# chu-tianxiang/QuIP-for-all

Hardware: AMD Instinct MI355X
Metric: decode tokens/sec bs=1 Llama-7B E8P12 2-bit, 1xMI355X; % HBM roofline (higher is better)
Workload: dtype i8xi8->i32 (fp16 I/O); 1 GPU; Llama-2-7B E8P12 random-init, bs=1 greedy decode, 1 hipGraph replay per token, positions [5, 833) of a 2048-slot static KV cache; layers=32, hidden=4096, ffn=11008, vocab=32000, parallelism=replicas x1 (no collective on the data path)

## Files before the change

quip_for_all_amd/csrc/decode_block.hip:

```cpp
#if defined(QUIP_POLL2) || defined(QUIP_POLL2_STAGGER) || defined(QUIP_ROWS_DIRECT) || defined(QUIP_MLP_PREFETCH) || defined(QUIP_INO_EXACT) || \
    defined(QUIP_QKV_ISSUE_EARLY) || defined(QUIP_OWNER_PREDECODE) || defined(QUIP_ATT_THREADS) || defined(QUIP_OHEAD)
#error "retired A/B switch (QUIP_POLL2, _POLL2_STAGGER, _ROWS_DIRECT, _MLP_PREFETCH, _INO_EXACT, _QKV_ISSUE_EARLY, _OWNER_PREDECODE, _ATT_THREADS, _OHEAD): the alternative was measured and its code removed; DESIGN.md 4.11 (QUIP_OHEAD: 4.13) has the result and the commit that still contains it"
#endif
#include "e8p_gemv_core.hip.h"
#include "attn_query.hip.h"
#include "engine_sync.hip.h"
#include "fht_wg512x.hip.h"
#include "token_tail.hip.h"
#include "block_engine_host.hip.h"

#ifndef QUIP_PREDECODE_DOWN
#define QUIP_PREDECODE_DOWN 2
#endif
#ifndef QUIP_PREDECODE_QKV
#define QUIP_PREDECODE_QKV 2
#endif
#ifndef QUIP_ATT_STAMPS
#define QUIP_ATT_STAMPS 0
#endif
#ifndef QUIP_MLP_STAMPS
#define QUIP_MLP_STAMPS 0
#endif
#if QUIP_MLP_STAMPS
#define MSTAMP(i) BSTAMP((i) < 7 ? 18 + (i) : 21 + (i))
#else
#define MSTAMP(i) do { } while (0)
#endif
#if QUIP_ATT_STAMPS
#define ASTAMP(i) BSTAMP(18 + (i))
#else
#define ASTAMP(i) do { } while (0)
#endif
#ifndef QUIP_WAIT_STAMPS
#define QUIP_WAIT_STAMPS 0
#endif
#if (QUIP_ATT_STAMPS != 0) + (QUIP_MLP_STAMPS != 0) + (QUIP_WAIT_STAMPS != 0) > 1
#error "QUIP_ATT_STAMPS, QUIP_MLP_STAMPS and QUIP_WAIT_STAMPS share the stamp slots 18..31: one at a time"
#endif
#if QUIP_WAIT_STAMPS == 1
#define WSTAMP(i) BSTAMP((i) < 7 ? 18 + (i) : 21 + (i))
#else
#define WSTAMP(i) do { } while (0)
#endif
#ifndef QUIP_NIB_PREDECODE_QKV
#define QUIP_NIB_PREDECODE_QKV 3
#endif
#ifndef QUIP_NIB_PREDECODE_GATE
#define QUIP_NIB_PREDECODE_GATE 3
#endif
#ifndef QUIP_NIB_PREDECODE_DOWN
#define QUIP_NIB_PREDECODE_DOWN 3
#endif
#ifndef QUIP_PREDECODE_GATE
#define QUIP_PREDECODE_GATE 2
#endif

namespace quip {

namespace {

using esync::u32x2_t;
using esync::u32x4_t;

struct BlockLayer {
  const uint4* W[7];
// ... 99 lines not shown
#if QUIP_BLOCK_G8
static_assert(BLds<24>::kBytes <= 160 * 1024 && BLds<4>::kBytes <= 160 * 1024, "LDS budget");
#else
static_assert(BLds<4>::kBytes <= 160 * 1024 && BLds<24>::kBytes <= 160 * 1024 && BLds<16>::kBytes <= 160 * 1024 && BLds<64>::kBytes <= 160 * 1024 &&
              BLds<16, true>::kBytes <= 160 * 1024 && BLds<64, true>::kBytes <= 160 * 1024 && BLds<12, true>::kBytes <= 160 * 1024,
              "LDS budget");
#endif

template <int REP, bool RVQ = false, bool HI = false>
__global__ __launch_bounds__(kThreads) void decode_block_kernel(BlockArgs a) {
  static_assert(!HI || (RVQ && Lds<REP>::kD4), "HI = virtual rows of twice the width on the D4 table mode");
  constexpr bool R3 = Lds<REP>::kRvq3;
  static_assert(!R3 || (RVQ && !HI), "RVQ3B: the virtual rows of RVQ");
  using slot_t = std::conditional_t<R3, u32x3, u32x4>;
  constexpr uint32_t PB = R3 ? 12u : 16u;
  extern __shared__ __attribute__((aligned(16))) char smem[];
  using B = BLds<REP, RVQ>;
  constexpr int VM = B::VM, KV = B::KV;
  constexpr int kRowU4V = VM * kRowU4, kRowU4DV = VM * kRowU4D;
  constexpr int kRowB = kRowU4V * 16;
  using T = Lds<REP>;
  int tid = threadIdx.x, lane = tid & 63;
  const int wave = __builtin_amdgcn_readfirstlane(tid >> 6);
  const int w = blockIdx.x;
  const int mgu = w >> 7;
  int n = lane & 15, q = lane >> 4;
  uint32_t* ctl = reinterpret_cast<uint32_t*>(a.ws + kWsCtl);
  uint64_t* zbufs = reinterpret_cast<uint64_t*>(a.ws + kWsZ);
  uint64_t* inbox = reinterpret_cast<uint64_t*>(a.ws + kWsInbox);
  uint64_t* frow = reinterpret_cast<uint64_t*>(a.ws + kWsRows);
  uint64_t* pbuf = reinterpret_cast<uint64_t*>(a.ws + kWsPart);
  int dbg_on = 0;
  const bool dbg_rt = (a.dbg_layer & 0x10000) != 0;
#define BSTAMP(i) do { if (dbg_on && tid == 0) a.dbg[w * 32 + (i)] = dbg_rt ? __builtin_amdgcn_s_memrealtime() : __builtin_amdgcn_s_memtime(); } while (0)

  slot_t qa[NSLOT], qb[NSLOT];
  uint32_t vo_row, vo_q[3], vo_gu[G8 ? 7 : FRB], vo_d[G8 ? 4 : 3], vo_d2b, vo_dr[3];
  const int qb0 = w < 128 ? 2 * w : 128 + w, qcnt = w < 128 ? 2 : 1;
  auto qmat = [](int b) { return b < 256 ? 0 : (b < 320 ? 1 : 2); };
  auto qblk = [](int b) { return b < 256 ? b : (b < 320 ? b - 256 : b - 320); };
  uint32_t lane_c, lane_c2, lane_c3 = 0u, xlane;
  constexpr bool NIB = T::kNib;
  constexpr bool kOHead = !RVQ;
  constexpr int kPreW = NIB ? 16 : 32;
  constexpr int kUnsc = T::kD4 ? 1 : (NIB ? 5 : 2);
  NibLane nlf = {0, 0, 0u};
  auto rederive = [&]() {
    int t = threadIdx.x;
    asm volatile("" : "+v"(t));
    tid = t; lane = t & 63; n = lane & 15; q = lane >> 4;
    vo_row = (uint32_t)((w * RPW + n) * kRowU4V + wave * 8 + q) * PB;
    if constexpr (G8) {
#pragma unroll
      for (int i = 0; i < 2; ++i) {
        const int bq = qb0 + (i < qcnt ? i : 0);
        vo_q[i] = (uint32_t)((qblk(bq) * 16 + n) * kRowU4V + wave * 8 + q) * PB;
      }
      vo_q[2] = vo_q[0];
#pragma unroll
      for (int i = 0; i < 7; ++i) {
        const int r = 16 * i + n, c = r >= FK ? 1 : 0, k = r - FK * c;
        vo_gu[i] = (uint32_t)((k * FL + 2 * (w & 127) + c) * kRowU4V + wave * 8 + q) * PB;
      }
#pragma unroll
      for (int i = 0; i < 4; ++i) {
        const int sl0 = i * kWaves + wave;
        const int sl = sl0 < JD ? sl0 : 0;
        vo_d[i] = (uint32_t)(((w * RPW + n) * kRowU4D + sl * 8 + q) * 16);
      }
      vo_d2b = 0u;
    } else if constexpr (TILED) {
      static_assert(!TILED || (!RVQ && PB == 16u), "the launch-tiled layout: plain E8P12 rows");
      constexpr int C = kRowU4V / 4, CD = kRowU4D / 4;
      const uint32_t lo = (uint32_t)lane * 16u;
      vo_row = (uint32_t)((w * C + 2 * wave) * 1024) + lo;
#pragma unroll
      for (int i = 0; i < 3; ++i) vo_q[i] = (uint32_t)((((3 * w + i) & 255) * C + 2 * wave) * 1024) + lo;
// ... 162 lines not shown
    h_in = a.tail.embed + (size_t)(tk >= 0 && tk < (long long)a.tail.vocab ? tk : 0) * HID;
  }
#pragma unroll
  for (int k = 0; k < 8; ++k)
    asm volatile("global_load_ushort %0, %1, off" : "=v"(hraw[k]) : "v"(reinterpret_cast<const uint16_t*>(h_in) + tid + 512 * k) : "memory");
  {
    const BlockLayer& L0 = a.layers[0];
    if constexpr (RVQ) ISSUE_RVQ_QKV(L0); else if constexpr (G8) { ISSUE8_QKV(L0, 0); ISSUE8_QKV(L0, 1); } else { ISSUE(L0, 0); ISSUE(L0, 1); ISSUE(L0, 2); }
  }
  constexpr int NQ = RVQ ? 12 : (G8 ? 4 : 6);
  int* accs = reinterpret_cast<int*>(smem + B::kAcc);
  for (int i = tid; i < B::kAccRows * 4; i += kThreads) accs[i] = 0;
  asm volatile("s_waitcnt vmcnt(%2)" : "+v"(tsrc), "+v"(tsrc3) : "n"(9 + NQ) : "memory");
  if constexpr (NIB) fill_tables_nib(tsrc, lane, wave);
  else fill_tables_from_lane<REP>(smem, tsrc, lane, wave);
  fill_t3_from_lane<REP>(smem, tsrc3, lane, wave);
  asm volatile("s_waitcnt vmcnt(%1)" : "+v"(gen) : "n"(8 + NQ) : "memory");
  const uint32_t ebase = ((uint32_t)__builtin_amdgcn_readfirstlane((int)gen) + 1u) << 10;
  asm volatile("s_waitcnt vmcnt(%8)" : "+v"(hraw[0]), "+v"(hraw[1]), "+v"(hraw[2]), "+v"(hraw[3]), "+v"(hraw[4]), "+v"(hraw[5]),
               "+v"(hraw[6]), "+v"(hraw[7]) : "n"(NQ) : "memory");
#pragma unroll
  for (int j = 0; j < 4; ++j) hreg[j] = (hraw[2 * j] & 0xffffu) | (hraw[2 * j + 1] << 16);
  const long long pos64 = *a.pos;
  const bool pos_ok = pos64 >= 0 && pos64 < (long long)a.max_len;
  const int pos = pos_ok ? (int)pos64 : 0;
  if (tid < 2 * HD)
    reinterpret_cast<float*>(smem + B::kCs)[tid] = (tid < HD ? a.cos : a.sin - HD)[(size_t)pos * HD + tid];
  had::wg_barrier<true>();
  uint32_t hop = 0;

  float* red = reinterpret_cast<float*>(smem + B::kRed);
  int* shs = reinterpret_cast<int*>(smem + B::kRed + 256);

  auto gather = [&](auto nv_tag, auto slots, int first, uint32_t tag, uint32_t code, float (&out)[decltype(nv_tag)::value][8]) {
    constexpr int NV = decltype(nv_tag)::value;
    u32x4_t p[2 * NV];
    uint32_t spins = 0;
    const uint64_t* src = zbufs + (size_t)first * 2048 + 4 * tid;
    for (;;) {
#pragma unroll
      for (int c = 0; c < NV; ++c) {
        esync::ld16(p[2 * c], src + c * 2048);
        esync::ld16(p[2 * c + 1], src + c * 2048 + 2);
      }
      esync::drain();
      bool ok = true;
#pragma unroll
      for (int j = 0; j < 2 * NV; ++j) {
        esync::own(p[j]);
        ok = ok && p[j].y == tag && p[j].w == tag;
      }
      if (esync::spin_step(ok, spins, ctl + 1, code + (uint32_t)w)) break;
    }
#pragma unroll
    for (int c = 0; c < NV; ++c)
      had::unpack8(make_uint4(p[2 * c].x, p[2 * c].z, p[2 * c + 1].x, p[2 * c + 1].z), out[c]);
    own_slots(slots);
  };
  auto publish16 = [&](int vec, int gr0, int row0, int sh, uint32_t tag) {
    if (tid < 8) {
      const int* s3 = accs + (row0 + 2 * tid) * 4;
      const float us = unscale_of(sh, kUnsc);
      const float f0 = __builtin_fmaf((float)s3[0], 65536.f, __builtin_fmaf((float)s3[1], 256.f, (float)s3[2]));
      const float f1 = __builtin_fmaf((float)s3[4], 65536.f, __builtin_fmaf((float)s3[5], 256.f, (float)s3[6]));
      esync::st_granule(zbufs + (size_t)vec * 2048 + gr0 + tid, pack_f16(f0 * us, f1 * us), tag);
    }
  };
  auto zero_acc = [&](int row0, int rows) {
    for (int i = tid; i < rows * 4; i += kThreads) accs[row0 * 4 + i] = 0;
  };

  constexpr bool E2 = B::kTwoBuf;
  float* xbuf = reinterpret_cast<float*>(smem + B::kBuf0);
  float* xbuf1 = reinterpret_cast<float*>(smem + B::kBuf1);
  auto planes_nat = [&](const float (&v)[8], float scale, int sh, uint32_t base) {
#pragma clang fp contract(off)
    const float p2 = as_f32((uint32_t)(sh + 127) << 23);
    const float s2 = had::fmul(scale, p2);
    const float va[4] = {v[0], v[1], v[2], v[3]}, vb[4] = {v[4], v[5], v[6], v[7]};
    if constexpr (HI) {
      const float e0[4] = {v[0], v[2], 0.f, 0.f}, e1[4] = {v[4], v[6], 0.f, 0.f}, e2[4] = {v[1], v[3], 0.f, 0.f}, e3[4] = {v[5], v[7], 0.f, 0.f};
      uint32_t dg[3][4];
      hadw::digit_words_magic(e0, s2, dg[0][0], dg[1][0], dg[2][0]);
      hadw::digit_words_magic(e1, s2, dg[0][1], dg[1][1], dg[2][1]);
      hadw::digit_words_magic(e2, s2, dg[0][2], dg[1][2], dg[2][2]);
      hadw::digit_words_magic(e3, s2, dg[0][3], dg[1][3], dg[2][3]);
#pragma unroll
      for (int d = 0; d < 3; ++d)
        *reinterpret_cast<uint4*>(smem + base + d * 2 * HID + 16 * tid) = make_uint4(dg[d][0], dg[d][1], dg[d][2], dg[d][3]);
    } else if constexpr (RVQ) {
// ... 1 lines not shown
      uint32_t dg[3][4];
      hadw::digit_words_magic(va, s2r, dg[0][0], dg[1][0], dg[2][0]);
      hadw::digit_words_magic(vb, s2r, dg[0][1], dg[1][1], dg[2][1]);
      hadw::digit_words_magic(va, s2, dg[0][2], dg[1][2], dg[2][2]);
      hadw::digit_words_magic(vb, s2, dg[0][3], dg[1][3], dg[2][3]);
#pragma unroll
      for (int d = 0; d < 3; ++d)
        *reinterpret_cast<uint4*>(smem + base + d * 2 * HID + 16 * tid) = make_uint4(dg[d][0], dg[d][1], dg[d][2], dg[d][3]);
    } else {
      uint32_t dg[3][2];
      hadw::digit_words_magic(va, s2, dg[0][0], dg[1][0], dg[2][0]);
      hadw::digit_words_magic(vb, s2, dg[0][1], dg[1][1], dg[2][1]);
#pragma unroll
      for (int d = 0; d < 3; ++d) {
        if constexpr (NIB) {
          *reinterpret_cast<uint32_t*>(smem + base + d * B::PSH + 4 * tid) = dg[d][0];
          *reinterpret_cast<uint32_t*>(smem + base + d * B::PSH + B::HOH + 4 * tid) = dg[d][1];
        } else {
          *reinterpret_cast<uint2*>(smem + base + d * HID + 8 * tid) = make_uint2(dg[d][0], dg[d][1]);
        }
      }
    }
  };
  auto norm_shift = [&](float sumsq_x, float scale) -> int {
    const float bound = sqrtf(sumsq_x) * 64.f * fabsf(scale) * 1.0625f;
    return had::shift_for(bound * ((RVQ && !HI) ? fmaxf(1.f, fabsf(a.resid_scale)) : 1.f));
  };
  auto red_sum8 = [&](int at) -> float {
    float r = red[at];
#pragma unroll
    for (int i = 1; i < 8; ++i) r = had::fadd(r, red[at + i]);
    return r;
  };
  auto edge = [&](auto z_tag, auto nc_tag, auto slots, int zvec, uint32_t tag, uint32_t code, const f16* sv_prev, const f16* ln,
                  const f16* su0, const f16* su1, float sc0, float sc1, bool two, auto after_gather, auto drip1, auto drip2, int sb) {
#if QUIP_ATT_STAMPS || QUIP_MLP_STAMPS || QUIP_WAIT_STAMPS
#define ESTAMP(i) do { } while (0)
#else
#define ESTAMP(i) do { if (sb >= 0) BSTAMP(sb + (i) + ((sb == 23 && (i) >= 2) ? 3 : 0)); } while (0)
#endif
    constexpr int NC = decltype(nc_tag)::value;
    constexpr bool HAVE_Z = decltype(z_tag)::value;
    u32x4 psv, pln, psu0, psu1;
    if constexpr (HAVE_Z) psv = *reinterpret_cast<const u32x4*>(sv_prev + 8 * tid);
    if constexpr (NC > 0) {
      pln = *reinterpret_cast<const u32x4*>(ln + 8 * tid);
      psu0 = *reinterpret_cast<const u32x4*>(su0 + 8 * tid);
      psu1 = *reinterpret_cast<const u32x4*>(su1 + 8 * tid);
    }
    auto u4 = [](const u32x4& v) { return make_uint4(v.x, v.y, v.z, v.w); };
    if constexpr (HAVE_Z) {
      float v[1][8];
      gather(std::integral_constant<int, 1>{}, slots, zvec, tag, code, v);
      asm volatile("" : "+v"(psv));
      if constexpr (NC > 0) asm volatile("" : "+v"(pln), "+v"(psu0), "+v"(psu1));
      after_gather();
      ESTAMP(0);
      hadw::fwd<12, 1, true, !E2>(v, xbuf, tid);
      ESTAMP(1);
      float svf[8];
      had::unpack8(u4(psv), svf);
#pragma unroll
      for (int j = 0; j < 4; ++j) {
        const f16x2 hh = as_f16x2(hreg[j]);
        const f16 n0 = had::out_elem(v[0][2 * j], 1.f / 64.f, true, svf[2 * j], false, 0.f, true, (float)hh.x);
        const f16 n1 = had::out_elem(v[0][2 * j + 1], 1.f / 64.f, true, svf[2 * j + 1], false, 0.f, true, (float)hh.y);
        hreg[j] = (uint32_t)__builtin_bit_cast(uint16_t, n0) | ((uint32_t)__builtin_bit_cast(uint16_t, n1) << 16);
      }
      drip1();
    }
    if constexpr (NC > 0) {
      float e[8];
#pragma unroll
      for (int j = 0; j < 4; ++j) {
        const f16x2 hh = as_f16x2(hreg[j]);
        e[2 * j] = (float)hh.x;
        e[2 * j + 1] = (float)hh.y;
      }
      float ssw = 0.f;
      {
#pragma clang fp contract(off)
#pragma unroll
        for (int r = 0; r < 8; ++r) ssw = __builtin_fmaf(e[r], e[r], ssw);
      }
      had::mul8(e, u4(pln));
      const int lane_ = tid & 63;
// ... 199 lines not shown
      had::wg_barrier<true>();
      ++hop;
      const int sh_lo = shs[0], sh_hi = shs[1];
      publish16(qc_lo, qblk(qb0) * 8, 0, sh_lo, ebase | hop);
      if (qcnt == 2) publish16(qc_hi, qblk(qb0 + 1) * 8, 16, qc_hi == qc_lo ? sh_lo : sh_hi, ebase | hop);
      had::wg_barrier<true>();
      zero_acc(0, 48);
      BSTAMP(3);
      return;
    }
    {
      const uint32_t x0 = xlane + (uint32_t)((((3 * w) >> 8) == c_lo ? 0 : 1) * 3 * B::PSH);
      const uint32_t x1 = xlane + (uint32_t)((((3 * w + 1) >> 8) == c_lo ? 0 : 1) * 3 * B::PSH);
      const uint32_t x2 = xlane + (uint32_t)((((3 * w + 2) >> 8) == c_lo ? 0 : 1) * 3 * B::PSH);
      if constexpr (decltype(pre_tag)::value) run_items3_pre(std::integral_constant<int, NPQ>{}, preq, 0, x0, x1, x2, 0);
      else run_items3(0, x0, x1, x2, 0);
      if constexpr (RVQ) run_items3(3, x0 + 4096u, x1 + 4096u, x2 + 4096u, 0);
    }
    had::wg_barrier<true>();
    ++hop;
    const int sh_lo = shs[0], sh_hi = shs[1];
#pragma unroll
    for (int i = 0; i < 3; ++i) {
      const int rbq = 3 * w + i, ci = rbq >> 8;
      publish16(ci, (rbq & 255) * 8, i * 16, ci == c_lo ? sh_lo : sh_hi, ebase | hop);
    }
    had::wg_barrier<true>();
    zero_acc(0, 48);
    BSTAMP(3);
  };
  {
    rederive();
    const int c_lo = qc_lo, c_hi = qc_hi;
    edge(std::false_type{}, std::integral_constant<int, 2>{}, SLOTS(M_QKV), -1, 0u, 0u, nullptr, Ld.ln[0], Ld.su[c_lo], Ld.su[c_hi],
         Ld.sc[c_lo], Ld.sc[c_hi], c_hi != c_lo, [&]() {}, [&]() {}, [&]() {}, -1);
    uint32_t none[NPQ][kPreW];
    P1_products(std::false_type{}, none);
  }
  for (int l = 0; l < a.n_layers; ++l) {
    dbg_on = a.dbg != nullptr && l == (a.dbg_layer & 0xffff);
    rederive();
    BSTAMP(0);
    if (tid < 64)
      reinterpret_cast<uint32_t*>(smem + B::kDescN)[tid] = reinterpret_cast<const uint32_t*>(a.layers + (l + 1 < a.n_layers ? l + 1 : l))[tid];
    if constexpr (RVQ) ISSUE_RVQ_O(Ld); else ISSUE(Ld, 3);

    rederive();
    const bool split = pos >= kSplitPos;
    const int part = w & 7, nparts = split ? kParts : 1;
    const bool head_wg = part == 0;
    const int hd = w >> 3;
    if (head_wg || split) {
      float c8[8], s8[8];
      const int d0 = (tid & 15) * 8;
      constexpr int ATH = 256;
      constexpr int LPK = HD / 8, NG = ATH / LPK, U = (RVQ && !HI && !R3) ? 2 : 4;
      constexpr int NST = ATH / 64;
      const int g = (tid & (ATH - 1)) / LPK;
      const int kvh = hd / GQH;
      const f16* kc = Ld.kcache + (size_t)kvh * a.max_len * HD;
      const f16* vc = Ld.vcache + (size_t)kvh * a.max_len * HD;
      uint4 kr0[U], vr0[U], kr1[U], vr1[U];
      const attn::CachedRows<HD, U, NG> rows{kc, vc, part, nparts, pos, d0};
      if (tid < ATH) {
        rows.load_round(kr0, vr0, g);
        if (part + nparts * NG * U < pos) rows.load_round(kr1, vr1, g + NG * U);
      }
      uint32_t svp_raw = 0u;
// ... 323 lines not shown
        if constexpr (RVQ) ISSUE_RVQ_GATE_G(Ld, 2); else if constexpr (G8) ISSUE8_GU(Ld, 2); else ISSUE(Ld, 6);
        if constexpr (HI) had8::planes_scatter_hi(v[0], sco, sh, reinterpret_cast<uint8_t*>(smem + B::kArea), tid);
        else if constexpr (RVQ) had8::planes_scatter_rvq(v[0], sco, a.resid_scale, sh, reinterpret_cast<uint8_t*>(smem + B::kArea), tid);
        else if constexpr (NIB) {
#pragma clang fp contract(off)
          const float s2 = had::fmul(sco, as_f32((uint32_t)(sh + 127) << 23));
          uint8_t* pb = reinterpret_cast<uint8_t*>(smem + B::kArea) + nib_half_of(tid) * B::HOH + nib_byte_of(tid);
#pragma unroll
          for (int k = 0; k < 8; ++k) {
            const int X = (int)__builtin_rintf(v[0][k] * s2);
            const int X1 = (X + 128) >> 8;
            const int H = (X1 + 128) >> 8;
            uint8_t* p = pb + 256 * k;
            p[0] = (uint8_t)H;
            p[B::PSH] = (uint8_t)X1;
            p[2 * B::PSH] = (uint8_t)X;
          }
        }
        else had8::planes_scatter(v[0], sco, sh, reinterpret_cast<uint8_t*>(smem + B::kArea), tid);
        if (tid == 0) shs[3] = sh;
        had::wg_barrier<true>();
      }
    }
    BSTAMP(8);
    if constexpr (RVQ) {
      run_item(6, xlane, 48);
      run_item(7, xlane + 4096u, 48);
    } else {
      if constexpr (NIB) { Frag Fo; frags(xlane, Fo); add_rows(mul_pre(Bon, Fo), 48); }
      else add_rows(item_multiply(Bo, xlane), 48);
    }
    had::wg_barrier<true>();
    ++hop;
    publish16(4, w * 8, 48, shs[3], ebase | hop);
    had::wg_barrier<true>();
    zero_acc(48, 16);
    BSTAMP(9);

    rederive();
#if QUIP_PREDECODE_GATE
    uint32_t Bg[kPreG][kPreW];
    if constexpr (!RVQ) {
      esync::drain();
      own_slots(SLOTS(M_GATE));
#pragma unroll
      for (int i = 0; i < kPreG; ++i) decode_pre(i, Bg[i]);
    }
#endif
    constexpr int HPIECES = B::kHadElems / 8, NHP = (HPIECES + kThreads - 1) / kThreads, OPIECES = RPO * 3 * (FL / 8);
    static_assert(OPIECES <= kThreads, "one piece of the owner vectors per thread");
    u32x4 fim[NHP], ovec = {0u, 0u, 0u, 0u};
#pragma unroll
    for (int i = 0; i < NHP; ++i) {
      const int pi = tid + kThreads * i;
      fim[i] = reinterpret_cast<const u32x4*>(Ld.had3)[pi < HPIECES ? pi : tid];
    }
    if (w < NRO) {
      const int p = tid < OPIECES ? tid : 0;
      const int row = p / (3 * (FL / 8)), rem = p - row * (3 * (FL / 8));
      const int vsel = rem / (FL / 8), piece = rem - vsel * (FL / 8);
      const int kr = RPO * w + row < FK ? RPO * w + row : FK - 1;
      ovec = *reinterpret_cast<const u32x4*>((vsel == 0 ? Ld.sv[4] : (vsel == 1 ? Ld.sv[5] : Ld.su[6])) + (size_t)kr * FL + piece * 8);
    }
    auto land_mlp_vectors = [&]() {
#pragma unroll
      for (int i = 0; i < NHP; ++i) {
        asm volatile("" : "+v"(fim[i]));
        if (tid + kThreads * i < HPIECES) *reinterpret_cast<u32x4*>(smem + B::kHad + (tid + kThreads * i) * 16) = fim[i];
      }
      asm volatile("" : "+v"(ovec));
      if (w < NRO && tid < OPIECES) *reinterpret_cast<u32x4*>(smem + B::kStash + tid * 16) = ovec;
    };
    edge(std::true_type{}, std::integral_constant<int, 2>{}, SLOTS(M_GATE), 4, ebase | hop, 0x7000u, Ld.sv[3], Ld.ln[1], Ld.su[4 + mgu], Ld.su[4 + mgu], Ld.sc[4 + mgu], Ld.sc[4 + mgu], false,
         [&]() { land_mlp_vectors(); BSTAMP(10); if constexpr (RVQ) ISSUE_RVQ_UP_A_G(Ld, 0); else if constexpr (G8) { ISSUE8_GU(Ld, 3); ISSUE8_GU(Ld, 4); } else ISSUE(Ld, 7); },
         [&]() { if constexpr (RVQ) ISSUE_RVQ_UP_A_G(Ld, 1); else if constexpr (G8) ISSUE8_GU(Ld, 5); else ISSUE(Ld, 8); },
         [&]() { if constexpr (RVQ) ISSUE_RVQ_UP_A_G(Ld, 2); else if constexpr (G8) ISSUE8_GU(Ld, 6); else ISSUE(Ld, 9); }, 18);
    BSTAMP(11);
    MSTAMP(0);
    if constexpr (RVQ || G8) {
      esync::drain();
      own_slots(SLOTS(M_GATE | M_UP));
    }
    MSTAMP(1);
    static_assert(FRB == 3, "three row blocks per matrix");
    if constexpr (RVQ) {
      const uint32_t xu = xlane;
      run_items3(0, xlane, xlane, xlane, 64);
      ISSUE_RVQ_UP_B(Ld);
      run_items3(3, xlane + 4096u, xlane + 4096u, xlane + 4096u, 64);
      run_items3(6, xu, xu, xu, 64 + 16 * FRB);
      esync::drain();
      own_slots(SLOTS(0x007u));
      run_items3(0, xu + 4096u, xu + 4096u, xu + 4096u, 64 + 16 * FRB);
    } else {
      if constexpr (G8) {
        Frag A;
        frags(xlane, A);
#if QUIP_PREDECODE_GATE
#define PRE_G(i) ((i) < kPreG ? Bg[(i) < kPreG ? (i) : 0] : nullptr)
#else
#define PRE_G(i) nullptr
#endif
        add_rows(item_vs(std::integral_constant<int, 0>{}, PRE_G(0), A), B::AGU);
        add_rows(item_vs(std::integral_constant<int, 1>{}, PRE_G(1), A), B::AGU + 16);
        MSTAMP(2);
        add_rows(item_vs(std::integral_constant<int, 2>{}, nullptr, A), B::AGU + 32);
        add_rows(item_vs(std::integral_constant<int, 3>{}, nullptr, A), B::AGU + 48);
        ISSUE8_DOWN(Ld, 0); ISSUE8_DOWN(Ld, 1); ISSUE8_DOWN(Ld, 2); ISSUE8_DOWN(Ld, 3);
        add_rows(item_vs(std::integral_constant<int, 4>{}, nullptr, A), B::AGU + 64);
// ... 42 lines not shown
      if (tid < 16 * NGU) {
        const int m = G8 ? (tid >= FK ? 1 : 0) : tid / 48, k = G8 ? tid - FK * m : tid - 48 * m;
        const int* s3 = accs + (B::AGU + tid) * 4;
        const float f = __builtin_fmaf((float)s3[0], 65536.f, __builtin_fmaf((float)s3[1], 256.f, (float)s3[2]));
        zcol[m * B::KP16 + (k & 3) * (B::KP16 / 4) + (k >> 2)] = (float)(f16)(f * unscale_of(shs[0], kUnsc));
      }
      had::wg_barrier<true>();
      zero_acc(B::AGU, 16 * NGU);
      ++hop;
      const uint32_t tag1 = ebase | hop;
      {
        const int o = tid >> 2, part = tid & 3;
        const int m = o & 1, kq = o >> 1;
        const bool live = kq < FK;
        const f16* hs = reinterpret_cast<const f16*>(smem + B::kHad) + mgu * B::KKP + (live ? kq : 0) * FK;
        constexpr int K4 = (FK + 3) / 4, KQ = B::KP16 / 4;
        static_assert(B::kZcol % 16 == 0 && KQ % 4 == 0 && K4 <= KQ, "a residue's z values: whole 16-byte pieces");
        float zz[KQ];
#pragma unroll
        for (int i = 0; i < (K4 + 3) / 4; ++i) {
          const float4 z4 = *reinterpret_cast<const float4*>(zcol + m * B::KP16 + part * KQ + 4 * i);
          zz[4 * i] = z4.x; zz[4 * i + 1] = z4.y; zz[4 * i + 2] = z4.z; zz[4 * i + 3] = z4.w;
        }
        float t = 0.f;
#pragma unroll
        for (int k4 = 0; k4 < K4; ++k4) {
          const int k = 4 * k4 + part;
          if (k < FK) t = __builtin_fmaf((float)hs[k], zz[k4], t);
        }
        t += __shfl_xor(t, 1, 64);
        t += __shfl_xor(t, 2, 64);
        t *= kMixScale;
        const float tn = __shfl_down(t, 4, 64);
        if (live && part == 0 && m == 0)
          esync::st_granule2(inbox + (((size_t)kq * 2 + mgu) * FL + 2 * (w & 127)), as_u32(t), as_u32(tn), tag1);
      }
      ++hop;
      const uint32_t tag2 = ebase | hop;
      BSTAMP(13);
#if QUIP_PREDECODE_DOWN
      uint32_t Bd[kPreD][kPreW];
      if constexpr (!RVQ) {
        esync::drain();
        own_slots(SLOTS(M_DOWN));
#pragma unroll
        for (int i = 0; i < kPreD; ++i) decode_pre(SDf(i), Bd[i]);
      }
#endif
      if (w < NRO) {
        const int rw = wave & (RPO - 1);
        const bool act = wave < RPO;
        const bool row_ok = RPO * w + rw < FK;
        auto fht256 = [&](auto& x) {
#pragma clang fp contract(off)
          constexpr int N = sizeof(x) / sizeof(float);
#pragma unroll
          for (int g = 0; g < N; g += 4) {
            const float a0 = x[g] + x[g + 1], a1 = x[g] - x[g + 1], a2 = x[g + 2] + x[g + 3], a3 = x[g + 2] - x[g + 3];
            x[g] = a0 + a2; x[g + 2] = a0 - a2; x[g + 1] = a1 + a3; x[g + 3] = a1 - a3;
          }
          hadw::lane_stages<N, 0, 6>(x, lane);
        };
        const f16* vecs = reinterpret_cast<const f16*>(smem + B::kStash) + (row_ok ? rw : 0) * 3 * FL;
        uint32_t* stage = reinterpret_cast<uint32_t*>(smem + B::kStage);
        if (act) {
          float v[8];
          {
            u32x4_t pc[4];
            const uint64_t* src = inbox + (((size_t)(RPO * w + (row_ok ? rw : 0)) * 2) * FL + 4 * lane);
            uint32_t spins = 0;
            for (;;) {
#pragma unroll
              for (int j = 0; j < 4; ++j) esync::ld16(pc[j], src + (j >> 1) * FL + 2 * (j & 1));
              esync::drain();
              bool ok = true;
#pragma unroll
              for (int j = 0; j < 4; ++j) {
                esync::own(pc[j]);
                ok = ok && (!row_ok || (pc[j].y == tag1 && pc[j].w == tag1));
              }
              if (esync::spin_step(ok, spins, ctl + 1, 0x1000u + (uint32_t)w)) break;
            }
            if (dbg_on && tid == 0) a.dbg[w * 32 + 25] = __builtin_amdgcn_s_memtime();
#pragma unroll
            for (int j = 0; j < 4; ++j) {
              v[2 * j] = row_ok ? __builtin_bit_cast(float, (uint32_t)pc[j].x) : 0.f;
              v[2 * j + 1] = row_ok ? __builtin_bit_cast(float, (uint32_t)pc[j].z) : 0.f;
            }
          }
          MSTAMP(4);
          fht256(v);
          float svf[8];
#pragma unroll
          for (int mh = 0; mh < 2; ++mh) {
            const uint2 svp = *reinterpret_cast<const uint2*>(vecs + mh * FL + lane * 4);
            const f16x2 s01 = as_f16x2(svp.x), s23 = as_f16x2(svp.y);
            svf[4 * mh] = (float)s01.x; svf[4 * mh + 1] = (float)s01.y; svf[4 * mh + 2] = (float)s23.x; svf[4 * mh + 3] = (float)s23.y;
          }
          float o[8];
#pragma unroll
          for (int r = 0; r < 8; ++r) o[r] = (float)had::out_elem(v[r], 1.f / 16.f, true, svf[r], false, 0.f, false, 0.f);
          MSTAMP(5);
          MSTAMP(6);
          const uint2 sup = *reinterpret_cast<const uint2*>(vecs + 2 * FL + lane * 4);
          const f16x2 s01 = as_f16x2(sup.x), s23 = as_f16x2(sup.y);
          const float suf[4] = {(float)s01.x, (float)s01.y, (float)s23.x, (float)s23.y};
          float e[4];
#pragma unroll
          for (int r = 0; r < 4; ++r) e[r] = had::fmul(had::fmul(o[4 + r], had::silu(o[r])), suf[r]);
          fht256(e);
          constexpr float kPre = 1.f / 16.f;
          uint16_t* stage16 = reinterpret_cast<uint16_t*>(stage);
#pragma unroll
          for (int r = 0; r < 4; ++r)
            stage16[(4 * lane + r) * RPO + rw] = __builtin_bit_cast(uint16_t, (f16)(e[r] * kPre));
        }
        MSTAMP(7);
        had::wg_barrier<true>();
        if (tid < FL / 2) {
          static_assert(RPO == 2, "one fp16 pair per column and owner");
          const uint2 d = *reinterpret_cast<const uint2*>(stage + 2 * tid);
          esync::st_granule2(frow + ((size_t)w * FL + 2 * tid), d.x, d.y, tag2);
        }
      }
      BSTAMP(14);
      typedef _Float16 f16x4 __attribute__((ext_vector_type(4)));
      constexpr int KCT = B::KP16 / 16;
      u32x2_t arow[2][KCT];
      {
        static_assert(NRO % 2 == 0 && NRO > 8 * (KCT - 1) && NRO <= 8 * KCT, "only q groups of the last k step are beyond the owners");
        if (wave == 0) {
          uint32_t spins0 = 0;
          const uint64_t* last = frow + ((size_t)(lane < NRO ? lane : 0) * FL + (FL - 1 - (w & 7)));
          for (;;) {
            u32x2_t f;
            esync::ld8(f, last);
            esync::drain();
            esync::own(f);
            if (esync::spin_step(f.y == tag2, spins0, ctl + 1, 0x3000u + (uint32_t)w)) break;
          }
        }
        had::wg_barrier<true>();
        BSTAMP(26);
        const bool beyond = 8 * (KCT - 1) + 2 * q >= NRO;
        const uint32_t vo_r = (uint32_t)((2 * q * FL + 16 * wave + n) * 8), vo_rl = (uint32_t)(((beyond ? 0 : 2 * q) * FL + 16 * wave + n) * 8);
        u32x2_t g[2][KCT][2];
        uint32_t spins = 0;
        for (;;) {
#pragma unroll
          for (int s = 0; s < KCT; ++s) {
            const char* base = reinterpret_cast<const char*>(frow) + (size_t)s * 8 * FL * 8;
// ... 166 lines not shown
          const int sl = i * kWaves + wave;
          if (sl < JD) {
#if QUIP_PREDECODE_DOWN
            if (i < kPreD) {
              const uint32_t* bs = Bd[i < kPreD ? i : 0];
              if constexpr (NIB) {
                Frag Fd;
                frags_d(xlane_d + (uint32_t)sl * kSliceD, Fd);
                add_rows(mul_pre(bs, Fd), B::AD);
              } else {
                i32x4 Bt[8];
#pragma unroll
                for (int t = 0; t < 8; ++t) Bt[t] = i32x4{(int)bs[4 * t], (int)bs[4 * t + 1], (int)bs[4 * t + 2], (int)bs[4 * t + 3]};
                add_rows(item_multiply<272>(Bt, xlane_d + (uint32_t)(sl * 544)), B::AD);
              }
              continue;
            }
#endif
            if constexpr (NIB) {
              Frag Fd;
              frags_d(xlane_d + (uint32_t)sl * kSliceD, Fd);
              add_rows(mul_slot(qa[SDf(i)], qb[SDf(i)], Fd), B::AD);
            } else {
              ItemAddr ad;
              item_addresses<REP>(qa[SDf(i)], qb[SDf(i)], lane_c, lane_c2, ad, lane_c3);
              add_rows(T::kD4 ? item_mfma_d4<272>(ad, xlane_d + (uint32_t)(sl * 544)) : item_mfma<272, R3>(ad, xlane_d + (uint32_t)(sl * 544)), B::AD);
            }
          }
        }
      }
      WSTAMP(8);
      had::wg_barrier<true>();
      ++hop;
      publish16(5, w * 8, B::AD, sh_d, ebase | hop);
      had::wg_barrier<true>();
      zero_acc(B::AD, 16);
      BSTAMP(17);
    }
    sv_d_prev = Ld.sv[6];
    const bool more = l + 1 < a.n_layers;
    if (more) {
      had::wg_barrier<true>();
      if (tid < 64) reinterpret_cast<uint32_t*>(smem + B::kDesc)[tid] = reinterpret_cast<const uint32_t*>(a.layers + l + 1)[tid];
      had::wg_barrier<true>();
    }
    rederive();
    uint32_t Bq[NPQ][kPreW];
    if constexpr (kPreQkv) {
#pragma unroll
      for (int i = 0; i < NPQ; ++i) decode_pre(SQf(i), Bq[i]);
    }
    {
      const int c_lo = qc_lo, c_hi = qc_hi;
      edge(std::true_type{}, std::integral_constant<int, 2>{}, SLOTS(0u), 5, ebase | hop, 0x4000u, sv_d_prev, Ld.ln[0], Ld.su[c_lo], Ld.su[c_hi],
           Ld.sc[c_lo], Ld.sc[c_hi], c_hi != c_lo,
           [&]() { BSTAMP(1); if constexpr (RVQ) { ISSUE_RVQ_QKV_G(Ld, 0); ISSUE_RVQ_QKV_G(Ld, 1); } else if constexpr (!kPreQkv) { ISSUE(Ld, 0); ISSUE(Ld, 1); } },
           [&]() { if constexpr (RVQ) ISSUE_RVQ_QKV_G(Ld, 2); else if constexpr (!kPreQkv) ISSUE(Ld, 2); }, [&]() {}, 23);
      BSTAMP(2);
    }
    if (more) P1_products(std::integral_constant<bool, kPreQkv>{}, Bq);
    esync::drain();
    own_slots(SLOTS(M_QKV));
  }
  if (whole_token) {
    static_assert(B::kArea % 16 == 0 && B::kAreaBytes >= tail::kLdsBytes, "the tail's x and reduction slots in the transient area");
    const bool tst = a.dbg != nullptr && (a.dbg_layer & 0xffff) == a.n_layers;
    ++hop;
    tail::run(a.tail, hreg, smem + B::kArea, ctl, zbufs, ebase | hop, w, a.rms_eps, pos64, tst ? a.dbg + w * 32 : nullptr, dbg_rt);
  }
  if (w == 0) {
    uint32_t e, fp;
    esync::ld4(e, ctl + 1);
    esync::ld4(fp, ctl + 2);
    esync::drain();
    esync::own(e);
    esync::own(fp);
    const bool failed = __builtin_amdgcn_readfirstlane((int)e) != 0;
    if (a.h_out) {
#pragma unroll
      for (int j = 0; j < 4; ++j) {
        reinterpret_cast<uint16_t*>(a.h_out)[tid + 512 * (2 * j)] = failed ? (uint16_t)0x7e00 : (uint16_t)(hreg[j] & 0xffffu);
        reinterpret_cast<uint16_t*>(a.h_out)[tid + 512 * (2 * j + 1)] = failed ? (uint16_t)0x7e00 : (uint16_t)(hreg[j] >> 16);
      }
    }
    if (tid == 0) {
      if (failed && fp == 0u) esync::st_word(ctl + 2, (uint32_t)pos + 1u);
      esync::st_word(ctl, ebase >> 10);
      if (!failed && (ebase >> 10) >= (1u << 22) - 2u) esync::st_word(ctl + 1, 0xE000u);
    }
  }
#undef BSTAMP
#undef ISSUE
#undef GU_RB
#undef GU_OFF2
#undef GU_COL
#undef SLOTS
#undef OFFC
#undef ISSUE_RVQ_QKV
#undef ISSUE_RVQ_O
#undef ISSUE_RVQ_GATE
#undef ISSUE_RVQ_UP_A
#undef ISSUE_RVQ_UP_B
#undef ISSUE_RVQ_GATE_G
#undef ISSUE_RVQ_DOWN_G0
#undef ISSUE_RVQ_QKV_G
#undef ISSUE_RVQ_DOWN_G1
#undef ISSUE_RVQ_DOWN_G2
#undef ISSUE_RVQ_UP_A_G
#undef ISSUE_RVQ_DOWN
}

tail::Args tail_args(const BlockEngineArgs& in) {
  tail::Args t;
  if (!in.lm_head) return t;
  t.tok = reinterpret_cast<int64_t*>(in.tok);
  t.pos = reinterpret_cast<int64_t*>(const_cast<void*>(in.pos));
  t.embed = reinterpret_cast<const f16*>(in.embed);
  t.norm_w = reinterpret_cast<const f16*>(in.final_norm);
  t.lm_head = reinterpret_cast<const f16*>(in.lm_head);
  t.logits = reinterpret_cast<f16*>(in.logits);
  t.xnorm = reinterpret_cast<f16*>(in.xnorm);
  t.vocab = in.vocab;
  return t;
}
// ... 61 lines not shown
```

quip_for_all_amd/csrc/engine_sync.hip.h:

```cpp
#pragma once
#include <hip/hip_runtime.h>
#include <stdint.h>

namespace quip {
namespace esync {

typedef uint32_t u32x4_t __attribute__((ext_vector_type(4)));
typedef uint32_t u32x2_t __attribute__((ext_vector_type(2)));

constexpr uint32_t kSpinLimit = 1u << 21;

__device__ __forceinline__ void st_granule(void* p, uint32_t value, uint32_t tag) {
  const u32x2_t v = {value, tag};
  asm volatile("global_store_dwordx2 %0, %1, off sc1" : : "v"(p), "v"(v) : "memory");
}
__device__ __forceinline__ void st_granule2(void* p, uint32_t v0, uint32_t v1, uint32_t tag) {
  const u32x4_t v = {v0, tag, v1, tag};
  asm volatile("global_store_dwordx4 %0, %1, off sc1\n\ts_nop 1" : : "v"(p), "v"(v) : "memory");
}
__device__ __forceinline__ void st_payload16(void* p, const u32x4_t& v) {
  asm volatile("global_store_dwordx4 %0, %1, off sc1\n\ts_nop 1" : : "v"(p), "v"(v) : "memory");
}
__device__ __forceinline__ void st_word(void* p, uint32_t v) {
  asm volatile("global_store_dword %0, %1, off sc1" : : "v"(p), "v"(v) : "memory");
}
__device__ __forceinline__ void drain() { asm volatile("s_waitcnt vmcnt(0)" ::: "memory"); }
template <int N>
__device__ __forceinline__ void wait_all_but() {
  static_assert(N >= 0 && N < 64, "vmcnt is a six-bit counter");
  asm volatile("s_waitcnt vmcnt(%0)" : : "n"(N) : "memory");
}

__device__ __forceinline__ void ld16(u32x4_t& dst, const void* p) {
  asm volatile("global_load_dwordx4 %0, %1, off sc1" : "=v"(dst) : "v"(p) : "memory");
}
__device__ __forceinline__ void ld16_keep(u32x4_t& dst, const void* p) {
  asm volatile("global_load_dwordx4 %0, %1, off sc1" : "+v"(dst) : "v"(p) : "memory");
}
__device__ __forceinline__ void ld8(u32x2_t& dst, const void* p) {
  asm volatile("global_load_dwordx2 %0, %1, off sc1" : "=v"(dst) : "v"(p) : "memory");
}
template <int OFF, bool NOP = false>
__device__ __forceinline__ void ld8_at(u32x2_t& dst, const void* sbase, uint32_t voff) {
  if constexpr (NOP) asm volatile("s_nop 4\n\tglobal_load_dwordx2 %0, %1, %2 offset:%3 sc1" : "=v"(dst) : "v"(voff), "s"(sbase), "n"(OFF) : "memory");
  else asm volatile("global_load_dwordx2 %0, %1, %2 offset:%3 sc1" : "=v"(dst) : "v"(voff), "s"(sbase), "n"(OFF) : "memory");
}
__device__ __forceinline__ void ld4(uint32_t& dst, const void* p) {
  asm volatile("global_load_dword %0, %1, off sc1" : "=v"(dst) : "v"(p) : "memory");
}
template <typename T>
__device__ __forceinline__ void own(T& v) { asm volatile("" : "+v"(v)); }

__device__ __forceinline__ void pack20x2(float a, float b, uint32_t tag, uint32_t& w0, uint32_t& w1) {
  const uint32_t ea = (__builtin_bit_cast(uint32_t, a) >> 23) & 0xffu, eb = (__builtin_bit_cast(uint32_t, b) >> 23) & 0xffu;
  uint32_t e = ea > eb ? ea : eb;
  e = e < 19u ? 19u : e;
  const float sc = __builtin_bit_cast(float, (272u - (e > 254u ? 254u : e)) << 23);
  int ma = (int)__builtin_rintf(a * sc), mb = (int)__builtin_rintf(b * sc);
  ma = ma < -524287 ? -524287 : (ma > 524287 ? 524287 : ma);
  mb = mb < -524287 ? -524287 : (mb > 524287 ? 524287 : mb);
  w0 = ((uint32_t)ma & 0xfffffu) | ((uint32_t)mb << 20);
  w1 = (((uint32_t)mb >> 12) & 0xffu) | (e << 8) | ((tag & 0xffffu) << 16);
}
__device__ __forceinline__ void unpack20x2(uint32_t w0, uint32_t w1, float& a, float& b) {
  const uint32_t e = (w1 >> 8) & 0xffu;
  const float sc = e == 255u ? __builtin_bit_cast(float, 0x7fc00000u) : __builtin_bit_cast(float, (e - 18u) << 23);
  a = (float)((int)(w0 << 12) >> 12) * sc;
  b = (float)((int)(((w0 >> 20) | (w1 << 12)) << 12) >> 12) * sc;
}

// ... 21 lines not shown
```

Before: 979.3 tokens/s.

## Issue hand-off polls early, ahead of the last predecoded weight item

At three cross-workgroup hand-offs (z_o, the MLP inbox, z_d) the first poll load and the edge vector loads are now issued before the last weight item is predecoded. That decode work then overlaps the round-trip latency of the poll, and the spin loop is entered only if the first check fails. The change also reads the next layer descriptor from an LDS copy instead of global memory, and adds debug-only sleep injections. In exchange, registers stay live across the decode, and one early read can still come back stale and need a re-poll.

```diff
diff --git a/quip_for_all_amd/csrc/decode_block.hip b/quip_for_all_amd/csrc/decode_block.hip
--- a/quip_for_all_amd/csrc/decode_block.hip
+++ b/quip_for_all_amd/csrc/decode_block.hip
@@ -31,6 +31,7 @@
 #else
 #define ASTAMP(i) do { } while (0)
 #endif
+#define POLL_MARK(text) asm volatile("; handoff poll " text ::: "memory")
 #ifndef QUIP_WAIT_STAMPS
 #define QUIP_WAIT_STAMPS 0
 #endif
@@ -196,6 +197,12 @@
   uint64_t* pbuf = reinterpret_cast<uint64_t*>(a.ws + kWsPart);
   int dbg_on = 0;
   const bool dbg_rt = (a.dbg_layer & 0x10000) != 0;
+  const bool nap_rows = a.dbg != nullptr && (a.dbg_layer & 0x20000) != 0 && w < NRO;
+  const bool nap_wg0 = a.dbg != nullptr && (a.dbg_layer & 0x40000) != 0 && w == 0;
+  auto nap = [](bool on) {
+    if (on)
+      for (int i = 0; i < 6; ++i) __builtin_amdgcn_s_sleep(127);
+  };
 #define BSTAMP(i) do { if (dbg_on && tid == 0) a.dbg[w * 32 + (i)] = dbg_rt ? __builtin_amdgcn_s_memrealtime() : __builtin_amdgcn_s_memtime(); } while (0)
 
   slot_t qa[NSLOT], qb[NSLOT];
@@ -207,6 +214,7 @@
   constexpr bool NIB = T::kNib;
   constexpr bool kOHead = !RVQ;
   constexpr int kPreW = NIB ? 16 : 32;
+  constexpr bool kEarly = NIB && !G8 && !RVQ;
   constexpr int kUnsc = T::kD4 ? 1 : (NIB ? 5 : 2);
   NibLane nlf = {0, 0, 0u};
   auto rederive = [&]() {
@@ -435,17 +443,19 @@
   float* red = reinterpret_cast<float*>(smem + B::kRed);
   int* shs = reinterpret_cast<int*>(smem + B::kRed + 256);
 
-  auto gather = [&](auto nv_tag, auto slots, int first, uint32_t tag, uint32_t code, float (&out)[decltype(nv_tag)::value][8]) {
+  auto z_request = [&](auto nv_tag, int first, auto& p) {
     constexpr int NV = decltype(nv_tag)::value;
-    u32x4_t p[2 * NV];
+    const uint64_t* src = zbufs + (size_t)first * 2048 + 4 * tid;
+#pragma unroll
+    for (int c = 0; c < NV; ++c) {
+      esync::ld16(p[2 * c], src + c * 2048);
+      esync::ld16(p[2 * c + 1], src + c * 2048 + 2);
+    }
+  };
+  auto gather_from = [&](auto nv_tag, auto early_tag, auto slots, int first, uint32_t tag, uint32_t code, auto& p, float (&out)[decltype(nv_tag)::value][8]) {
+    constexpr int NV = decltype(nv_tag)::value;
     uint32_t spins = 0;
-    const uint64_t* src = zbufs + (size_t)first * 2048 + 4 * tid;
-    for (;;) {
-#pragma unroll
-      for (int c = 0; c < NV; ++c) {
-        esync::ld16(p[2 * c], src + c * 2048);
-        esync::ld16(p[2 * c + 1], src + c * 2048 + 2);
-      }
+    auto check = [&]() -> bool {
       esync::drain();
       bool ok = true;
 #pragma unroll
@@ -453,12 +463,23 @@
         esync::own(p[j]);
         ok = ok && p[j].y == tag && p[j].w == tag;
       }
-      if (esync::spin_step(ok, spins, ctl + 1, code + (uint32_t)w)) break;
-    }
+      return esync::spin_step(ok, spins, ctl + 1, code + (uint32_t)w);
+    };
+    bool through = false;
+    if constexpr (decltype(early_tag)::value) through = check();
+    if (!through)
+      for (;;) {
+        z_request(nv_tag, first, p);
+        if (check()) break;
+      }
 #pragma unroll
     for (int c = 0; c < NV; ++c)
       had::unpack8(make_uint4(p[2 * c].x, p[2 * c].z, p[2 * c + 1].x, p[2 * c + 1].z), out[c]);
     own_slots(slots);
+  };
+  auto gather = [&](auto nv_tag, auto slots, int first, uint32_t tag, uint32_t code, float (&out)[decltype(nv_tag)::value][8]) {
+    u32x4_t p[2 * decltype(nv_tag)::value];
+    gather_from(nv_tag, std::false_type{}, slots, first, tag, code, p, out);
   };
   auto publish16 = [&](int vec, int gr0, int row0, int sh, uint32_t tag) {
     if (tid < 8) {
@@ -526,8 +547,18 @@
     for (int i = 1; i < 8; ++i) r = had::fadd(r, red[at + i]);
     return r;
   };
+  struct EdgeIn { u32x4 psv, pln, psu0, psu1; u32x4_t p[2]; };
+  auto edge_vectors = [&](auto z_tag, auto nc_tag, const f16* sv_prev, const f16* ln, const f16* su0, const f16* su1, EdgeIn& in) {
+    if constexpr (decltype(z_tag)::value) in.psv = *reinterpret_cast<const u32x4*>(sv_prev + 8 * tid);
+    if constexpr (decltype(nc_tag)::value > 0) {
+      in.pln = *reinterpret_cast<const u32x4*>(ln + 8 * tid);
+      in.psu0 = *reinterpret_cast<const u32x4*>(su0 + 8 * tid);
+      in.psu1 = *reinterpret_cast<const u32x4*>(su1 + 8 * tid);
+    }
+  };
   auto edge = [&](auto z_tag, auto nc_tag, auto slots, int zvec, uint32_t tag, uint32_t code, const f16* sv_prev, const f16* ln,
-                  const f16* su0, const f16* su1, float sc0, float sc1, bool two, auto after_gather, auto drip1, auto drip2, int sb) {
+                  const f16* su0, const f16* su1, float sc0, float sc1, bool two, auto after_gather, auto drip1, auto drip2, int sb,
+                  auto early_tag, EdgeIn& in) {
 #if QUIP_ATT_STAMPS || QUIP_MLP_STAMPS || QUIP_WAIT_STAMPS
 #define ESTAMP(i) do { } while (0)
 #else
@@ -535,17 +566,14 @@
 #endif
     constexpr int NC = decltype(nc_tag)::value;
     constexpr bool HAVE_Z = decltype(z_tag)::value;
-    u32x4 psv, pln, psu0, psu1;
-    if constexpr (HAVE_Z) psv = *reinterpret_cast<const u32x4*>(sv_prev + 8 * tid);
-    if constexpr (NC > 0) {
-      pln = *reinterpret_cast<const u32x4*>(ln + 8 * tid);
-      psu0 = *reinterpret_cast<const u32x4*>(su0 + 8 * tid);
-      psu1 = *reinterpret_cast<const u32x4*>(su1 + 8 * tid);
-    }
+    constexpr bool EARLY = decltype(early_tag)::value;
+    static_assert(!EARLY || (HAVE_Z && NC > 0), "an early poll: of an edge behind a hand-off");
+    if constexpr (!EARLY) edge_vectors(z_tag, nc_tag, sv_prev, ln, su0, su1, in);
+    u32x4 &psv = in.psv, &pln = in.pln, &psu0 = in.psu0, &psu1 = in.psu1;
     auto u4 = [](const u32x4& v) { return make_uint4(v.x, v.y, v.z, v.w); };
     if constexpr (HAVE_Z) {
       float v[1][8];
-      gather(std::integral_constant<int, 1>{}, slots, zvec, tag, code, v);
+      gather_from(std::integral_constant<int, 1>{}, early_tag, slots, zvec, tag, code, in.p, v);
       asm volatile("" : "+v"(psv));
       if constexpr (NC > 0) asm volatile("" : "+v"(pln), "+v"(psu0), "+v"(psu1));
       after_gather();
@@ -811,8 +839,9 @@
   {
     rederive();
     const int c_lo = qc_lo, c_hi = qc_hi;
+    EdgeIn ein0;
     edge(std::false_type{}, std::integral_constant<int, 2>{}, SLOTS(M_QKV), -1, 0u, 0u, nullptr, Ld.ln[0], Ld.su[c_lo], Ld.su[c_hi],
-         Ld.sc[c_lo], Ld.sc[c_hi], c_hi != c_lo, [&]() {}, [&]() {}, [&]() {}, -1);
+         Ld.sc[c_lo], Ld.sc[c_hi], c_hi != c_lo, [&]() {}, [&]() {}, [&]() {}, -1, std::false_type{}, ein0);
     uint32_t none[NPQ][kPreW];
     P1_products(std::false_type{}, none);
   }
@@ -1202,6 +1231,7 @@
     }
     had::wg_barrier<true>();
     ++hop;
+    nap(nap_wg0);
     publish16(4, w * 8, 48, shs[3], ebase | hop);
     had::wg_barrier<true>();
     zero_acc(48, 16);
@@ -1210,12 +1240,16 @@
     rederive();
 #if QUIP_PREDECODE_GATE
     uint32_t Bg[kPreG][kPreW];
+    constexpr int kAheadO = 1;
+    static_assert(!kEarly || kPreG > kAheadO, "the early poll of z_o goes out in front of an item decoded ahead");
     if constexpr (!RVQ) {
       esync::drain();
       own_slots(SLOTS(M_GATE));
 #pragma unroll
-      for (int i = 0; i < kPreG; ++i) decode_pre(i, Bg[i]);
-    }
+      for (int i = 0; i < kPreG - (kEarly ? kAheadO : 0); ++i) decode_pre(i, Bg[i]);
+    }
+#else
+    static_assert(!kEarly, "the early poll of z_o needs an item decoded ahead");
 #endif
     constexpr int HPIECES = B::kHadElems / 8, NHP = (HPIECES + kThreads - 1) / kThreads, OPIECES = RPO * 3 * (FL / 8);
     static_assert(OPIECES <= kThreads, "one piece of the owner vectors per thread");
@@ -1241,10 +1275,23 @@
       asm volatile("" : "+v"(ovec));
       if (w < NRO && tid < OPIECES) *reinterpret_cast<u32x4*>(smem + B::kStash + tid * 16) = ovec;
     };
+    EdgeIn eo;
+#if QUIP_PREDECODE_GATE
+    if constexpr (kEarly) {
+      edge_vectors(std::true_type{}, std::integral_constant<int, 2>{}, Ld.sv[3], Ld.ln[1], Ld.su[4 + mgu], Ld.su[4 + mgu], eo);
+      POLL_MARK("z_o: request");
+      z_request(std::integral_constant<int, 1>{}, 4, eo.p);
+      POLL_MARK("z_o: last item");
+#pragma unroll
+      for (int i = kPreG - kAheadO; i < kPreG; ++i) decode_pre(i, Bg[i]);
+      POLL_MARK("z_o: check");
+    }
+#endif
     edge(std::true_type{}, std::integral_constant<int, 2>{}, SLOTS(M_GATE), 4, ebase | hop, 0x7000u, Ld.sv[3], Ld.ln[1], Ld.su[4 + mgu], Ld.su[4 + mgu], Ld.sc[4 + mgu], Ld.sc[4 + mgu], false,
          [&]() { land_mlp_vectors(); BSTAMP(10); if constexpr (RVQ) ISSUE_RVQ_UP_A_G(Ld, 0); else if constexpr (G8) { ISSUE8_GU(Ld, 3); ISSUE8_GU(Ld, 4); } else ISSUE(Ld, 7); },
          [&]() { if constexpr (RVQ) ISSUE_RVQ_UP_A_G(Ld, 1); else if constexpr (G8) ISSUE8_GU(Ld, 5); else ISSUE(Ld, 8); },
-         [&]() { if constexpr (RVQ) ISSUE_RVQ_UP_A_G(Ld, 2); else if constexpr (G8) ISSUE8_GU(Ld, 6); else ISSUE(Ld, 9); }, 18);
+         [&]() { if constexpr (RVQ) ISSUE_RVQ_UP_A_G(Ld, 2); else if constexpr (G8) ISSUE8_GU(Ld, 6); else ISSUE(Ld, 9); }, 18,
+         std::integral_constant<bool, kEarly>{}, eo);
     BSTAMP(11);
     MSTAMP(0);
     if constexpr (RVQ || G8) {
@@ -1353,25 +1400,63 @@
         t += __shfl_xor(t, 2, 64);
         t *= kMixScale;
         const float tn = __shfl_down(t, 4, 64);
+        nap(nap_wg0);
         if (live && part == 0 && m == 0)
           esync::st_granule2(inbox + (((size_t)kq * 2 + mgu) * FL + 2 * (w & 127)), as_u32(t), as_u32(tn), tag1);
       }
       ++hop;
       const uint32_t tag2 = ebase | hop;
       BSTAMP(13);
+      constexpr int kAheadI = 1;
+      static_assert(!kEarly || kPreD > kAheadI, "the early poll of the inbox goes out in front of an item decoded ahead");
+      const int rw = wave & (RPO - 1);
+      const bool row_ok = RPO * w + rw < FK;
+      u32x4_t pc[4];
+      uint32_t ispins = 0;
+      bool inbox_in = false;
+      auto inbox_src = [&]() -> const uint64_t* { return inbox + (((size_t)(RPO * w + (row_ok ? rw : 0)) * 2) * FL + 4 * lane); };
+      auto inbox_request = [&]() {
+        const uint64_t* src = inbox_src();
+#pragma unroll
+        for (int j = 0; j < 4; ++j) esync::ld16(pc[j], src + (j >> 1) * FL + 2 * (j & 1));
+      };
+      auto inbox_tags = [&]() -> bool {
+        bool ok = true;
+#pragma unroll
+        for (int j = 0; j < 4; ++j) {
+          esync::own(pc[j]);
+          ok = ok && (!row_ok || (pc[j].y == tag1 && pc[j].w == tag1));
+        }
+        return ok;
+      };
+      auto inbox_check = [&]() -> bool {
+        esync::drain();
+        return esync::spin_step(inbox_tags(), ispins, ctl + 1, 0x1000u + (uint32_t)w);
+      };
 #if QUIP_PREDECODE_DOWN
       uint32_t Bd[kPreD][kPreW];
       if constexpr (!RVQ) {
         esync::drain();
         own_slots(SLOTS(M_DOWN));
 #pragma unroll
-        for (int i = 0; i < kPreD; ++i) decode_pre(SDf(i), Bd[i]);
-      }
+        for (int i = 0; i < kPreD - (kEarly ? kAheadI : 0); ++i) decode_pre(SDf(i), Bd[i]);
+        if constexpr (kEarly) {
+          const bool ownw = w < NRO && wave < RPO;
+          POLL_MARK("inbox: request");
+          esync::ld16x4_if<16, FL * 8, FL * 8 + 16>(ownw, pc[0], pc[1], pc[2], pc[3], inbox_src());
+          POLL_MARK("inbox: last item");
+#pragma unroll
+          for (int i = kPreD - kAheadI; i < kPreD; ++i) decode_pre(SDf(i), Bd[i]);
+          POLL_MARK("inbox: check");
+          esync::drain();
+          inbox_in = ownw && __all(inbox_tags());
+        }
+      }
+#else
+      static_assert(!kEarly, "the early poll of the inbox needs an item decoded ahead");
 #endif
       if (w < NRO) {
-        const int rw = wave & (RPO - 1);
         const bool act = wave < RPO;
-        const bool row_ok = RPO * w + rw < FK;
         auto fht256 = [&](auto& x) {
 #pragma clang fp contract(off)
           constexpr int N = sizeof(x) / sizeof(float);
@@ -1387,21 +1472,11 @@
         if (act) {
           float v[8];
           {
-            u32x4_t pc[4];
-            const uint64_t* src = inbox + (((size_t)(RPO * w + (row_ok ? rw : 0)) * 2) * FL + 4 * lane);
-            uint32_t spins = 0;
-            for (;;) {
-#pragma unroll
-              for (int j = 0; j < 4; ++j) esync::ld16(pc[j], src + (j >> 1) * FL + 2 * (j & 1));
-              esync::drain();
-              bool ok = true;
-#pragma unroll
-              for (int j = 0; j < 4; ++j) {
-                esync::own(pc[j]);
-                ok = ok && (!row_ok || (pc[j].y == tag1 && pc[j].w == tag1));
+            if (!inbox_in)
+              for (;;) {
+                inbox_request();
+                if (inbox_check()) break;
               }
-              if (esync::spin_step(ok, spins, ctl + 1, 0x1000u + (uint32_t)w)) break;
-            }
             if (dbg_on && tid == 0) a.dbg[w * 32 + 25] = __builtin_amdgcn_s_memtime();
 #pragma unroll
             for (int j = 0; j < 4; ++j) {
@@ -1438,6 +1513,7 @@
         }
         MSTAMP(7);
         had::wg_barrier<true>();
+        nap(nap_rows);
         if (tid < FL / 2) {
           static_assert(RPO == 2, "one fp16 pair per column and owner");
           const uint2 d = *reinterpret_cast<const uint2*>(stage + 2 * tid);
@@ -1670,6 +1746,7 @@
       WSTAMP(8);
       had::wg_barrier<true>();
       ++hop;
+      nap(nap_wg0);
       publish16(5, w * 8, B::AD, sh_d, ebase | hop);
       had::wg_barrier<true>();
       zero_acc(B::AD, 16);
@@ -1679,21 +1756,34 @@
     const bool more = l + 1 < a.n_layers;
     if (more) {
       had::wg_barrier<true>();
-      if (tid < 64) reinterpret_cast<uint32_t*>(smem + B::kDesc)[tid] = reinterpret_cast<const uint32_t*>(a.layers + l + 1)[tid];
+      if (tid < 64) reinterpret_cast<uint32_t*>(smem + B::kDesc)[tid] = reinterpret_cast<const uint32_t*>(smem + B::kDescN)[tid];
       had::wg_barrier<true>();
     }
     rederive();
     uint32_t Bq[NPQ][kPreW];
+    constexpr int kAheadD = 1;
     if constexpr (kPreQkv) {
 #pragma unroll
-      for (int i = 0; i < NPQ; ++i) decode_pre(SQf(i), Bq[i]);
+      for (int i = 0; i < NPQ - (kEarly ? kAheadD : 0); ++i) decode_pre(SQf(i), Bq[i]);
+    }
+    EdgeIn eq;
+    if constexpr (kEarly) {
+      static_assert(!kEarly || (kPreQkv && NPQ > kAheadD), "the early poll of z_d goes out in front of an item decoded ahead");
+      edge_vectors(std::true_type{}, std::integral_constant<int, 2>{}, sv_d_prev, Ld.ln[0], Ld.su[qc_lo], Ld.su[qc_hi], eq);
+      POLL_MARK("z_d: request");
+      z_request(std::integral_constant<int, 1>{}, 5, eq.p);
+      POLL_MARK("z_d: last item");
+#pragma unroll
+      for (int i = NPQ - kAheadD; i < NPQ; ++i) decode_pre(SQf(i), Bq[i]);
+      POLL_MARK("z_d: check");
     }
     {
       const int c_lo = qc_lo, c_hi = qc_hi;
       edge(std::true_type{}, std::integral_constant<int, 2>{}, SLOTS(0u), 5, ebase | hop, 0x4000u, sv_d_prev, Ld.ln[0], Ld.su[c_lo], Ld.su[c_hi],
            Ld.sc[c_lo], Ld.sc[c_hi], c_hi != c_lo,
            [&]() { BSTAMP(1); if constexpr (RVQ) { ISSUE_RVQ_QKV_G(Ld, 0); ISSUE_RVQ_QKV_G(Ld, 1); } else if constexpr (!kPreQkv) { ISSUE(Ld, 0); ISSUE(Ld, 1); } },
-           [&]() { if constexpr (RVQ) ISSUE_RVQ_QKV_G(Ld, 2); else if constexpr (!kPreQkv) ISSUE(Ld, 2); }, [&]() {}, 23);
+           [&]() { if constexpr (RVQ) ISSUE_RVQ_QKV_G(Ld, 2); else if constexpr (!kPreQkv) ISSUE(Ld, 2); }, [&]() {}, 23,
+           std::integral_constant<bool, kEarly>{}, eq);
       BSTAMP(2);
     }
     if (more) P1_products(std::integral_constant<bool, kPreQkv>{}, Bq);
@@ -1728,6 +1818,7 @@
     }
   }
 #undef BSTAMP
+#undef POLL_MARK
 #undef ISSUE
 #undef GU_RB
 #undef GU_OFF2
diff --git a/quip_for_all_amd/csrc/engine_sync.hip.h b/quip_for_all_amd/csrc/engine_sync.hip.h
--- a/quip_for_all_amd/csrc/engine_sync.hip.h
+++ b/quip_for_all_amd/csrc/engine_sync.hip.h
@@ -36,6 +36,22 @@
 }
 __device__ __forceinline__ void ld16_keep(u32x4_t& dst, const void* p) {
   asm volatile("global_load_dwordx4 %0, %1, off sc1" : "+v"(dst) : "v"(p) : "memory");
+}
+template <int O1, int O2, int O3>
+__device__ __forceinline__ void ld16x4_if(bool on, u32x4_t& d0, u32x4_t& d1, u32x4_t& d2, u32x4_t& d3, const void* p) {
+  const uint32_t m = (uint32_t)__builtin_amdgcn_readfirstlane(on ? -1 : 0);
+  uint64_t keep;
+  asm volatile("s_mov_b64 %4, exec\n\t"
+               "s_and_b32 exec_lo, exec_lo, %5\n\t"
+               "s_and_b32 exec_hi, exec_hi, %5\n\t"
+               "global_load_dwordx4 %0, %6, off sc1\n\t"
+               "global_load_dwordx4 %1, %6, off offset:%7 sc1\n\t"
+               "global_load_dwordx4 %2, %6, off offset:%8 sc1\n\t"
+               "global_load_dwordx4 %3, %6, off offset:%9 sc1\n\t"
+               "s_mov_b64 exec, %4"
+               : "=&v"(d0), "=&v"(d1), "=&v"(d2), "=&v"(d3), "=&s"(keep)
+               : "s"(m), "v"(p), "n"(O1), "n"(O2), "n"(O3)
+               : "memory", "scc");
 }
 __device__ __forceinline__ void ld8(u32x2_t& dst, const void* p) {
   asm volatile("global_load_dwordx2 %0, %1, off sc1" : "=v"(dst) : "v"(p) : "memory");
```

Measured after the change: 997.9 tokens/s (median of 6 runs). +1.9%, better.
